# SCUT-CCNL/3DSIFT

Measured on AMD Instinct MI355X. Metric: Mvoxels/s end-to-end KpSiftAlgorithm on 512^3 fp32, higher is better.
Workload: dtype f32

## Files before the change

3dsift_amd/csrc/context.hip:

```cpp
#include <float.h>
#include <math.h>
#include <stdlib.h>
#include <string.h>

#include <algorithm>
#include <atomic>
#include <mutex>
#include <thread>

#include "ctx_internal.h"

#pragma clang fp contract(off)

namespace s3d {

static thread_local std::string g_last_error;
void set_last_error(const std::string &s) { g_last_error = s; }

int set_device(int device) {
	int n = 0;
	if (hipGetDeviceCount(&n) != hipSuccess || n <= 0) {
		set_last_error("no HIP device visible: this library has no CPU fallback");
		return SIFT3D_ERR_NO_DEVICE;
	}
// ... 31 lines not shown
		int *base = nullptr;
		S3D_HIP(hipMalloc(&base, sizeof(int) * words));
		hipError_t me = hipMemsetAsync(base, 0, sizeof(int) * words, c->stream);
		if (me == hipSuccess) me = hipStreamSynchronize(c->stream);
		if (me != hipSuccess) {
			hipFree(base);
			set_last_error(std::string("HIP error: ") + hipGetErrorString(me) + " (clearing the split-window scratch)");
			return SIFT3D_ERR_HIP;
		}
		c->dsplit.gacc = base;
		c->dsplit.gmass = reinterpret_cast<float *>(base + (size_t)scap * kDesc);
		c->dsplit.gdone = reinterpret_cast<unsigned *>(base + (size_t)scap * (kDesc + 8));
		c->dsplit.cap = scap;
	}
	S3D_HIP(hipMalloc(&c->d_prov, sizeof(unsigned) * ((size_t)c->ext_cap + 1)));
	c->det.prov = c->d_prov; c->det.prov_count = c->d_prov + c->ext_cap; c->det.prov_cap = c->ext_cap;
	if (c->det_o.size() > 1) {
		const size_t n2 = c->det_o.size() - 1;
		const unsigned slice = std::max(64u, (unsigned)(c->ext_cap / n2));
		S3D_HIP(hipMalloc(&c->d_prov2, sizeof(unsigned) * ((size_t)slice + 1) * n2));
		for (size_t o = 1; o < c->det_o.size(); o++) {
			c->det_o[o].prov = c->d_prov2 + (o - 1) * ((size_t)slice + 1);
			c->det_o[o].prov_count = c->det_o[o].prov + slice;
			c->det_o[o].prov_cap = slice;
		}
	}
	return SIFT3D_OK;
}

extern "C" void sift3d_default_params(sift3d_params *p) {
	if (!p) return;
	p->num_kp_levels = 3;
	p->sigma_default = 1.6f;
	p->sigma_n_default = 1.15f;
	p->peak_thresh = 0.1f;
	p->max_eig_thres = 0.9f;
	p->corner_thresh = 0.4f;
}
// ... 215 lines not shown
		CHECKED(hipMalloc(&c->arena, sizeof(float) * total));
	}
	float *p = c->arena;
	if (c->in_own) c->in.d = c->in_own;
	else { c->in.d = p; p += al64(c->in.n()); }
	c->tmpA.assign((size_t)std::max(1, c->noct), nullptr);
	c->tmpB.assign((size_t)std::max(1, c->noct), nullptr);
	for (int o = 0; o < c->noct && !c->slab; o++) {
		const size_t vo = al64(c->gss[(size_t)o * c->ng].n());
		c->tmpA[o] = p; p += vo;
		c->tmpB[o] = p; p += vo;
	}
	for (auto &L : c->gss) { L.d = p; p += al64(L.n()); }
	for (auto &L : c->dog) { L.d = p; p += al64(L.n()); }

	const size_t nwords = 1 + (size_t)std::max(1, c->noct * c->nd) + 8 + 1;
	CHECKED(hipMalloc(&c->d_words, sizeof(unsigned) * nwords));
	CHECKED(hipMemset(c->d_words, 0, sizeof(unsigned) * nwords));
	CHECKED(hipHostMalloc(&c->h_words, sizeof(unsigned) * 8, hipHostMallocDefault));
	CHECKED(hipMalloc(&c->d_slots_part, sizeof(unsigned) * slots_scratch_words()));
	c->d_inmax = c->d_words;
	c->d_dogmax = c->d_words + 1;
	c->d_total = c->d_words + 1 + std::max(1, c->noct * c->nd);
	c->d_nkp = c->d_total + 2;

	const int scan_planes = c->slab ? (c->own1 - c->own0) : cfg.nz;
	{
		const size_t kl = (size_t)c->p.num_kp_levels;
		const size_t words = kl * (size_t)scan_planes * cfg.ny * ((cfg.nx + 63) / 64);
		c->det_blocks = kl * (size_t)scan_planes * ((cfg.ny + 15) / 16);
		CHECKED(hipMalloc(&c->det.masks, sizeof(unsigned long long) * std::max<size_t>(words, 1)));
		CHECKED(hipMalloc(&c->det.block_counts, sizeof(unsigned) * std::max<size_t>(c->det_blocks, 1)));
		CHECKED(hipMalloc(&c->det.block_offsets, sizeof(unsigned) * std::max<size_t>(c->det_blocks, 1)));
	}
	c->det.total = c->d_total;
	{
		const bool det_serial = hook(SIFT3D_HOOK_DET_SERIAL) != 0;
		if (!c->slab && c->noct > 1 && !det_serial && c->ostream.size() > 1 && c->ostream[1] != c->stream) {
// ... 63 lines not shown
extern "C" int sift3d_create(sift3d_handle *out, const float *volume, int nx, int ny, int nz, const sift3d_params *params,
                             int device, int volume_on_device) {
	if (!out || !volume || nx <= 0 || ny <= 0 || nz <= 0) { set_last_error("sift3d_create: bad argument"); return SIFT3D_ERR_ARG; }
	if ((size_t)nx * ny * nz >= ((size_t)1 << 31)) { set_last_error("volume too large for int32 voxel indices"); return SIFT3D_ERR_ARG; }
	CreateCfg cfg;
	cfg.nx = nx; cfg.ny = ny; cfg.nz = nz;
	if (!volume_on_device) cfg.host_volume = volume;
	int rc = create_common(out, cfg, params, device);
	if (rc) return rc;
	sift3d_ctx *c = *out;
	const size_t V0 = (size_t)nx * ny * nz;
	hipError_t e = hipSuccess;
	if (volume_on_device) e = hipMemcpyAsync(c->in.d, volume, sizeof(float) * V0, hipMemcpyDeviceToDevice, c->stream);
	else if ((rc = join_upload(c)) != SIFT3D_OK) { sift3d_destroy(c); *out = nullptr; return rc; }
	if (e == hipSuccess) {
		unsigned *d_nonfinite = c->d_words + 1 + (size_t)std::max(1, c->noct * c->nd) + 8;
		launch_absmax(c->in.d, V0, c->d_inmax, c->stream, d_nonfinite);
		launch_scale_by_max(c->in.d, V0, c->d_inmax, c->stream);
		e = hipMemcpyAsync(&c->h_words[7], d_nonfinite, sizeof(unsigned), hipMemcpyDeviceToHost, c->stream);
		if (e == hipSuccess) e = hipStreamSynchronize(c->stream);
		if (e == hipSuccess && c->h_words[7] != 0) { c->nonfinite = true; c->use_fused = false; }
	}
	if (e == hipSuccess) e = hipGetLastError();
	if (e != hipSuccess) { set_last_error(hipGetErrorString(e)); sift3d_destroy(c); *out = nullptr; return SIFT3D_ERR_HIP; }
	return SIFT3D_OK;
}

#ifndef S3D_FUSED_MIN_DEFAULT
#define S3D_FUSED_MIN_DEFAULT 33
#endif
#ifndef S3D_O0_TAIL_SLOTS_DEFAULT
// ... 209 lines not shown

static int enqueue_detect(sift3d_ctx *c, const RunPlan &plan, int upto) {
	hipStream_t st = c->stream, sb = plan_stream(c, plan.det_two ? 1 : 0), sc = plan_stream(c, plan.det_rest_stream);
	std::vector<DetectLevels> DLs((size_t)c->noct);
	const int nl = c->nd - 2;
	const Taps *lt = c->g_last_elide ? &c->taps[c->ng - 1] : nullptr;
	DetectOpts dopt;
	dopt.neighbours = c->dopt.neighbours; dopt.refine = c->dopt.refine;
	dopt.max_offset = c->dopt.max_offset; dopt.contrast_thresh = c->dopt.contrast_thresh; dopt.edge_ratio = c->dopt.edge_ratio;
	const DetectOpts *dop = c->run_full ? &dopt : nullptr;
	if (upto >= 3)
		for (int o = 0; o < c->noct; o++) fill_detect_levels(c, o, DLs[(size_t)o]);
	auto bufs = [&](int o) -> const DetectBufs & { return plan.det_two && o > 0 ? c->det_o[(size_t)o] : c->det; };
	auto mark = [&](int o, hipStream_t s) {
		const Level &C = c->dog[(size_t)o * c->nd + 1];
		launch_detect_mark(DLs[(size_t)o], nl, C.nx, C.ny, C.zr_all(), c->p.peak_thresh, o + c->octave_base, bufs(o), s, lt, dop);
	};
	hipStream_t join = plan.det_early ? sb : st;
	if (plan.det_early) {
		S3D_HIP(hipEventRecord(c->ev_det_fork, st));
		mark(0, st);
		S3D_HIP(hipStreamWaitEvent(sb, c->ev_det_fork, 0));
	}
	for (int o = 1; o < c->noct; o++) S3D_HIP(hipStreamWaitEvent(join, c->ev_done[(size_t)o], 0));
	S3D_HIP(hipEventRecord(c->ev[1], join));
	S3D_HIP(hipEventRecord(c->ev[2], join));
	if (upto < 3) return SIFT3D_OK;
	if (plan.det_two) {
		for (int o = 1; o < c->noct; o++) {
			if (plan.det_rest_own && o >= 2) S3D_HIP(hipStreamWaitEvent(sc, c->ev_done[(size_t)o], 0));
			mark(o, o == 1 ? sb : sc);
// ... 7 lines not shown
		if (!plan.det_two) mark(o, st);
		if (plan.det_two && o == 1) {
			S3D_HIP(hipStreamWaitEvent(st, c->ev_det_join, 0));
			if (sc != sb) S3D_HIP(hipStreamWaitEvent(st, c->ev_det_join2, 0));
		}
		if (plan.emit == kEmitMultiAll || (plan.emit == kEmitMultiRest && o > 0)) multi.push_back(DetectEmitItem{&DLs[(size_t)o], nl, C.nx, C.ny, C.zr_all(), o + c->octave_base, &bufs(o)});
		else launch_detect_emit(DLs[(size_t)o], nl, C.nx, C.ny, C.zr_all(), o + c->octave_base, bufs(o), c->d_ext, c->ext_cap, st);
	}
	if (!multi.empty()) launch_detect_emit_multi(multi.data(), (int)multi.size(), c->d_ext, c->ext_cap, c->d_total, st);
	return SIFT3D_OK;
}

void enqueue_slots(sift3d_ctx *c) {
	launch_slots(c->d_ext, c->d_codes, c->d_total, c->ext_cap, c->d_nkp, c->d_order, c->kp_cap, c->d_slots_part, c->stream);
}
void enqueue_orient(sift3d_ctx *c, int rank, int world) {
	launch_orient(c->d_ext, c->d_codes, c->d_total, c->ext_cap, c->d_levels, c->d_luts, c->d_lutpool, c->p.max_eig_thres, c->p.corner_thresh,
	              rank, world, c->d_order, c->d_nkp + 3, c->stream);
	enqueue_slots(c);
}
void enqueue_describe(sift3d_ctx *c, int rank, int world, bool with_desc) {
	if (with_desc)
		launch_describe(c->d_ext, c->d_total, c->ext_cap, c->d_levels, c->d_luts, c->d_lutpool, c->d_desc, c->kp_cap, rank, world, c->d_order,
		                c->d_nkp, c->d_nkp + 1, c->stream, c->desc_lut_lds, &c->dsplit);
	launch_finalize(c->d_ext, c->d_total, c->ext_cap, with_desc, c->d_kpout, c->d_xyz, c->kp_cap, c->stream);
}

static int run_scratch(sift3d_ctx *c, int upto) {
	if (c->run_refine && upto >= 4 && c->refined_cap < c->kp_cap) {
		hipFree(c->d_refined); c->d_refined = nullptr; c->refined_cap = 0;
		S3D_HIP(hipMalloc(&c->d_refined, sizeof(sift3d_refined) * (size_t)c->kp_cap));
		c->refined_cap = c->kp_cap;
	}
	if (c->dsplit_dirty && c->dsplit.gacc) {
		S3D_HIP(hipMemsetAsync(c->dsplit.gacc, 0, sizeof(int) * (size_t)c->dsplit.cap * (kDesc + 8 + 1), c->stream));
		c->dsplit_dirty = false;
	}
	return SIFT3D_OK;
}

static int run_enqueue(sift3d_ctx *c, int upto, bool part_orient) {
	int rc = set_device(c->device);
	if (rc) return rc;
	if ((rc = run_scratch(c, upto)) != SIFT3D_OK) return rc;
	hipStream_t st = c->stream;
	const RunPlan &plan = c->plan;
	if (c->gate) { S3D_HIP(hipStreamWaitEvent(st, c->gate, 0)); c->gate = nullptr; }
	S3D_HIP(hipMemsetAsync(c->d_dogmax, 0, sizeof(unsigned) * (size_t)(std::max(1, c->noct * c->nd) + 6), st));
	S3D_HIP(hipEventRecord(c->ev[0], st));
	if ((rc = enqueue_pyramid(c, plan)) != SIFT3D_OK) return rc;
	if ((rc = enqueue_detect(c, plan, upto)) != SIFT3D_OK) return rc;
	S3D_HIP(hipEventRecord(c->ev[3], st));
	if (upto >= 4) enqueue_orient(c, part_orient ? c->part_rank : 0, part_orient ? c->part_world : 1);
	S3D_HIP(hipEventRecord(c->ev[4], st));
	if (upto >= 4) enqueue_describe(c, c->part_rank, c->part_world, upto >= 5);
	if (upto >= 4 && c->run_refine) {
		DogTable T;
		fill_dog_table(c, T);
		launch_refine(c->d_ext, c->d_total, c->ext_cap, c->kp_cap, T, c->p.num_kp_levels, c->d_refined, st);
	}
	S3D_HIP(hipEventRecord(c->ev[5], st));
	S3D_HIP(hipMemcpyAsync(c->h_words, c->d_total, sizeof(unsigned) * 5, hipMemcpyDeviceToHost, st));
	return SIFT3D_OK;
}


static int run_finish(sift3d_ctx *c, int upto, bool &again) {
	again = false;
	int rc = set_device(c->device);
	if (rc) return rc;
// ... 295 lines not shown
```

3dsift_amd/csrc/ctx_internal.h:

```cpp
#pragma once

#include <string>
#include <thread>
#include <vector>

#include "sift3d_internal.h"

using s3d::DescSplit; using s3d::DetectBufs; using s3d::DevKp; using s3d::Level; using s3d::LevelRef; using s3d::Taps; using s3d::WinLut;


constexpr int kChainStream = -1;
enum { kEmitPerOctave = 0, kEmitMultiRest = 1, kEmitMultiAll = 2 };
struct RunPlan {
	struct Oct {
		int head = 0, tail = 0;
		bool tail_moved = false;
		int prio = 0;
		int head_slots = 0, tail_slots = 0;
	};
	std::vector<Oct> oct;
	bool chain = false;
	int small_first = -1;
	s3d::SmallArgs small{};
	bool det_two = false;
// ... 26 lines not shown
	float *in_own = nullptr;
	void *in_raw = nullptr;
	hipStream_t up_stream = nullptr;
	std::thread uploader;
	int upload_rc = SIFT3D_OK;
	std::string upload_err;
	size_t arena_floats = 0;
	Level in;
	std::vector<Level> gss, dog;
	std::vector<float *> tmpA, tmpB;
	std::vector<hipStream_t> ostream;
	hipStream_t cstream = nullptr;
	std::vector<hipEvent_t> ev_seed, ev_done;
	hipEvent_t ev_fork = nullptr;
	unsigned *d_words = nullptr;
	unsigned *d_slots_part = nullptr;
	unsigned *h_words = nullptr;
	unsigned *d_inmax = nullptr, *d_dogmax = nullptr, *d_total = nullptr, *d_nkp = nullptr;
	DetectBufs det{};
	size_t det_blocks = 0;
	std::vector<DetectBufs> det_o;
	unsigned long long *d_masks2 = nullptr;
	unsigned *d_counts2 = nullptr, *d_offsets2 = nullptr, *d_prov2 = nullptr;
	hipEvent_t ev_det_fork = nullptr, ev_det_join = nullptr, ev_det_join2 = nullptr;
	DevKp *d_ext = nullptr;
	int *d_codes = nullptr, *d_order = nullptr;
	unsigned ext_cap = 0, kp_cap = 0;
	LevelRef *d_levels = nullptr;
	WinLut *d_luts = nullptr;
	float *d_lutpool = nullptr;
// ... 40 lines not shown
	size_t ext_arena_floats = 0;
};

namespace s3d {
bool build_taps(float sigma, Taps &t);
void level_sigmas(const sift3d_params &p, std::vector<float> &sig, float &base_sigma);
void build_faces(FaceConst *F);
bool build_facesym(const FaceConst *F, FaceSym *S);
bool append_lut(std::vector<float> &pool, WinLut &L, int which, float sigma, float radius, float u, float scale);
int set_device(int device);
int alloc_lists(sift3d_ctx *c, unsigned ext_cap);
float level_scale(const sift3d_params &p, int octave, int s);
void plan_pyramid(sift3d_ctx *c, int noct_total);
void fill_detect_levels(const sift3d_ctx *c, int o, DetectLevels &DL);
void enqueue_slots(sift3d_ctx *c);
void enqueue_orient(sift3d_ctx *c, int rank, int world);
void enqueue_describe(sift3d_ctx *c, int rank, int world, bool with_desc);
int upload_luts(sift3d_ctx *c, const std::vector<WinLut> &luts, std::vector<float> &pool);
std::vector<WinLut> blank_luts(const sift3d_ctx *c);
size_t arena_floats_of(const sift3d_ctx *c);
int create_common(sift3d_handle *out, const CreateCfg &cfg, const sift3d_params *params, int device);
int join_upload(sift3d_ctx *c);
int run_impl(sift3d_ctx *c, int upto, bool part_orient = false);
}
```

3dsift_amd/csrc/kernels_desc.hip:

```cpp
#include <float.h>

#include <stdio.h>

#include <algorithm>

#include "sift3d_internal.h"

namespace s3d {

__constant__ FaceConst c_faces[kFaces];
__constant__ FaceSym c_sym;

hipError_t upload_faces(const FaceConst *faces, const FaceSym *sym) {
	hipError_t e = hipMemcpyToSymbol(HIP_SYMBOL(c_faces), faces, sizeof(FaceConst) * kFaces);
	if (e == hipSuccess) e = hipMemcpyToSymbol(HIP_SYMBOL(c_sym), sym, sizeof(FaceSym));
	return e;
}

__device__ __forceinline__ void win_bounds_d(float c, float rad, float u, int n, int &lo, int &hi) {
	int s = (int)floorf(c - __fdiv_rn(rad, u));
	lo = s > 1 ? s : 1;
	int e = (int)ceilf(c + __fdiv_rn(rad, u));
	hi = e < (n - 2) ? e : n - 2;
}
// ... 822 lines not shown
	int total = 0;
	for (int i = 0; i < kDesc; i++) total += marks[i] != 0u;
	float n2 = 0.0f;
	for (int i = 0; i < total; i++) n2 = n2 + trunc_thresh * trunc_thresh;
	const float cn = (float)((double)sqrtf(n2) + DBL_EPSILON);
	const float cv = trunc_thresh * (float)(1.0 / (double)cn);
	for (int i = tid; i < kDesc; i += 256) row[i] = marks[i] != 0u ? cv : 0.0f;
}
void launch_describe_overflow(const DevKp *kps, unsigned k, const LevelRef *d_levels, const WinLut *d_luts, const float *d_lutpool, float *d_desc,
                              hipStream_t st) {
	hipLaunchKernelGGL(k_describe_overflow, dim3(1), dim3(256), 0, st, kps, k, d_levels, d_luts, d_lutpool, d_desc);
}

void launch_describe(const DevKp *kps, const unsigned *d_count, unsigned cap, const LevelRef *d_levels, const WinLut *d_luts,
                     const float *d_lutpool, float *d_desc, unsigned kp_cap, int part_rank, int part_world, const int *order,
                     const unsigned *d_nkp, unsigned *d_work, hipStream_t st, bool lut_in_lds, const DescSplit *split) {
	(void)hipMemsetAsync(d_work, 0, 2 * sizeof(unsigned), st);
	DescSplit sp{};
	if (split && split->gacc && lut_in_lds && !hook(SIFT3D_HOOK_DESC_NOSPLIT)) sp = *split;
	static const int desc_grid = dev_tune_i("S3D_DESC_GRID", 256 * 8);
	const int dev_flags = (hook(SIFT3D_HOOK_DESC_NOCACHE) ? 1 : 0) | (hook(SIFT3D_HOOK_DESC_EXACT_CELLS) ? 2 : 0) | (hook(SIFT3D_HOOK_DESC_MASS_SHIFT) & 63) << 8;
	const unsigned wide_hi = kWideBelow, wide_lo = sp.gacc ? std::min(kSplit4Below, wide_hi) : 0u;
	if (lut_in_lds) {
		hipLaunchKernelGGL((k_describe<true, 256>), dim3(desc_grid), dim3(256), 0, st, kps, d_count, cap, d_levels, d_luts, d_lutpool, d_desc, kp_cap,
		                   part_rank, part_world, order, d_nkp, d_work, dev_flags, wide_lo, wide_hi, sp, DescPartial{});
		if (wide_hi > wide_lo)
			hipLaunchKernelGGL((k_describe<true, 512>), dim3(256 * 2), dim3(512), 0, st, kps, d_count, cap, d_levels, d_luts, d_lutpool, d_desc, kp_cap,
			                   part_rank, part_world, order, d_nkp, d_work, dev_flags, wide_lo, wide_hi, DescSplit{}, DescPartial{});
	} else {
		hipLaunchKernelGGL((k_describe<false, 256>), dim3(256 * 8), dim3(256), 0, st, kps, d_count, cap, d_levels, d_luts, d_lutpool, d_desc, kp_cap,
		                   part_rank, part_world, order, d_nkp, d_work, dev_flags, 0u, 0u, DescSplit{}, DescPartial{});
	}
// ... 124 lines not shown
```

3dsift_amd/csrc/kernels_detect.hip:

```cpp
#include <stdio.h>
#include <string.h>
#include <stdlib.h>

#include <algorithm>

#include "sift3d_internal.h"

namespace s3d {

#ifndef S3D_DETDIAG
#define S3D_DETDIAG 0
#endif
constexpr int kRows = 32;
constexpr int kThreads = 256;

constexpr int kQueue = 640;
__global__ void __launch_bounds__(kThreads) k_mark(DetectLevels L, int nx, int ny, ZRange zr, int nyb, float peak_thresh,
                                                   unsigned long long *__restrict__ masks, unsigned *__restrict__ block_counts,
                                                   unsigned *__restrict__ prov, unsigned *__restrict__ prov_count, unsigned prov_cap,
                                                   unsigned *__restrict__ total) {
	__shared__ unsigned s_cnt[kThreads / 64];
	__shared__ uint2 s_q[kThreads / 64][kQueue];
	extern __shared__ unsigned long long s_mask_dyn[];
	const int segw = min((nx + 63) >> 6, 64);
	const int b = blockIdx.x;
	const int nz = zr.zo1 - zr.zo0;
	const int yb = b % nyb, zi = (b / nyb) % nz, lvl = b / (nyb * nz);
	const int z = zr.zo0 + zi;
	const int zg = z + zr.zoff;
	const float *__restrict__ cur = L.cur[lvl];
	const float *__restrict__ prev = L.prev[lvl];
	const float *__restrict__ next = L.next[lvl];
	const bool lazy_prev = lvl == 0 && L.prev0_hi != nullptr, lazy_next = lvl == L.nextl_slot && L.nextl_hi != nullptr;
	const bool lazy_g = lvl == L.nextl_slot && L.lazy_src != nullptr;
	const float thr = peak_thresh * __uint_as_float(*L.absmax_bits[lvl]);
	const int wpr = (nx + 63) >> 6;
	const int lane = threadIdx.x & 63, wid = threadIdx.x >> 6;
	const size_t sy = (size_t)nx, sz = (size_t)nx * ny;
	const bool z_in = (zg >= 1 && zg <= zr.nzg - 2);
	const int y0 = yb * kRows;
	constexpr int kBatch = 8;
	const int nrows = min(kRows, ny - y0);
	const int swid = __builtin_amdgcn_readfirstlane(wid);
	const int r_lo = swid * (kRows / 4), r_hi = min(nrows, (swid + 1) * (kRows / 4));
	uint2 *q = s_q[swid];
	unsigned long long *mloc = s_mask_dyn + (size_t)swid * (kRows / 4) * segw;
	for (int i = lane; i < (kRows / 4) * segw; i += 64) mloc[i] = 0ull;
	const unsigned long long lt = (1ull << lane) - 1ull;
	const size_t plane0 = sz * (size_t)z + sy * (size_t)y0;
	int qn = 0;
	auto evaluate = [&](int first, int n, int seg0) {
		if (S3D_DETDIAG & 1) {
			const uint2 qd = q[first + min(lane, n - 1)];
			if (lane < n && __uint_as_float(qd.x) == 12345.678f) atomicOr(&mloc[0], 1ull);
			return;
		}
// ... 26 lines not shown
					else total[1] = 1u;
				}
			}
			return;
		}
		const float n7 = lazy_next ? (L.nextl_hi[ic] - L.nextl_lo[ic]) * (-1.0f) : next[ic];
		const bool mn = !dmax && v < n0 && v < n5 && v < n6 && v < n7;
		const bool mx = dmax && v > n0 && v > n5 && v > n6 && v > n7;
		if (act && (mn || mx)) atomicOr(&mloc[rr * segw + xw], 1ull << bit);
	};
	unsigned cnt = 0;
	for (int seg0 = 0; seg0 < wpr; seg0 += 64) {
		const int seg1 = min(wpr, seg0 + 64);
		if (z_in) {
			const int ry_a = max(r_lo, 1 - y0), ry_b = min(r_hi, ny - 1 - y0);
			const int nws = seg1 - seg0;
			const float *__restrict__ pl = cur + sz * (size_t)z + (size_t)seg0 * 64;
			auto word = [&](float v, float u, float d, float xl, float xr, int wseg, unsigned idrow) {
				const float hi = fmaxf(fmaxf(u, d), fmaxf(xl, xr)), lo = fminf(fminf(u, d), fminf(xl, xr));
				const bool gmax = v > hi;
				const bool c = fabsf(v) > thr && (gmax || v < lo) && !((S3D_DETDIAG & 2) && v != 12345.678f);
				const unsigned long long m = __ballot(c);
				if (c) {
					const unsigned pos = __builtin_amdgcn_mbcnt_hi((unsigned)(m >> 32), __builtin_amdgcn_mbcnt_lo((unsigned)m, (unsigned)qn));
					q[pos] = make_uint2(__float_as_uint(v), idrow | (gmax ? 0x10000u : 0u) | (unsigned)(wseg << 6) | (unsigned)lane);
				}
				qn += (int)__popcll(m);
			};
			const unsigned omax = (unsigned)(nx - 1 - seg0 * 64);
			for (int w0 = 0; w0 < nws && ry_a < ry_b; w0 += kBatch) {
				unsigned off[kBatch];
#pragma unroll
				for (int bb = 0; bb < kBatch; bb++) off[bb] = min((unsigned)(min(w0 + bb, nws - 1) * 64 + lane), omax);
				const int eoff = (lane & 1) ? (int)min((unsigned)((w0 + kBatch) * 64), omax) : w0 * 64 - 1;
				float up[kBatch], mid[kBatch], emid;
				{
					const float *ra = pl + sy * (size_t)(y0 + ry_a - 1), *rb = ra + sy;
#pragma unroll
					for (int bb = 0; bb < kBatch; bb++) { up[bb] = ra[off[bb]]; mid[bb] = rb[off[bb]]; }
					emid = rb[eoff];
				}
				for (int ry = ry_a; ry < ry_b; ry++) {
					const float *rd = pl + sy * (size_t)(y0 + ry + 1);
					float dn[kBatch], xl[kBatch], xr[kBatch];
#pragma unroll
					for (int bb = 0; bb < kBatch; bb++) dn[bb] = rd[off[bb]];
					const float edn = rd[eoff];
#pragma unroll
					for (int bb = 0; bb < kBatch; bb++) {
						const int le = __builtin_amdgcn_readlane(__float_as_int(bb == 0 ? emid : mid[bb > 0 ? bb - 1 : 0]), bb == 0 ? 0 : 63);
						const int re = __builtin_amdgcn_readlane(__float_as_int(bb == kBatch - 1 ? emid : mid[bb < kBatch - 1 ? bb + 1 : 0]), bb == kBatch - 1 ? 1 : 0);
						xl[bb] = __int_as_float(__builtin_amdgcn_update_dpp(le, __float_as_int(mid[bb]), 0x138 , 0xf, 0xf, false));
						xr[bb] = __int_as_float(__builtin_amdgcn_update_dpp(re, __float_as_int(mid[bb]), 0x130 , 0xf, 0xf, false));
					}
					const unsigned idrow = (unsigned)((ry - r_lo) << 12);
#pragma unroll
					for (int bb = 0; bb < kBatch; bb++)
						if (w0 + bb < nws) word(mid[bb], up[bb], dn[bb], xl[bb], xr[bb], w0 + bb, idrow);
					while (qn >= 64) {
						qn -= 64;
						evaluate(qn, 64, seg0);
					}
#pragma unroll
					for (int bb = 0; bb < kBatch; bb++) { up[bb] = mid[bb]; mid[bb] = dn[bb]; }
					emid = edn;
				}
			}
		}
		if (qn > 0) evaluate(0, qn, seg0);
		qn = 0;
		for (int ry = r_lo; ry < r_hi; ry++) {
			unsigned long long *mrow = masks + ((size_t)(lvl * nz + zi) * ny + (y0 + ry)) * wpr;
			for (int xw = seg0 + lane; xw < seg1; xw += 64) {
				const unsigned long long m = mloc[(ry - r_lo) * segw + xw - seg0];
				mrow[xw] = m;
				cnt += (unsigned)__popcll(m);
				mloc[(ry - r_lo) * segw + xw - seg0] = 0ull;
			}
		}
	}
#pragma unroll
// ... 371 lines not shown
                                                   int octave, DetectLevels L, DevKp *__restrict__ out, unsigned cap,
                                                   unsigned *__restrict__ total) {
	__shared__ unsigned s_wave[kThreads / 64];
	emit_block((int)blockIdx.x, masks, block_offsets, nx, ny, zr, nyb, octave, L.level_id, L.scale, out, cap, total, s_wave);
}

__global__ void __launch_bounds__(kThreads) k_emit_multi(EmitMulti M, DevKp *__restrict__ out, unsigned cap, unsigned *__restrict__ total) {
	__shared__ unsigned s_wave[kThreads / 64];
	int k = 0;
	while (k + 1 < M.n && blockIdx.x >= M.o[k + 1].block0) k++;
	const EmitOct &E = M.o[k];
	emit_block((int)(blockIdx.x - E.block0), E.masks, E.offsets, E.nx, E.ny, E.zr, E.nyb, E.octave, E.level_id, E.scale, out, cap, total, s_wave);
}

void launch_detect_mark(const DetectLevels &L, int nlevels, int nx, int ny, const ZRange &zr, float peak_thresh, int octave,
                        const DetectBufs &b, hipStream_t st, const Taps *lazy_taps, const DetectOpts *opt) {
	if (opt) { launch_mark_full(L, nlevels, nx, ny, zr, kRows, peak_thresh, *opt, b, st); return; }
	const int nyb = (ny + kRows - 1) / kRows;
	const int nzl = zr.zo1 - zr.zo0;
	if (nzl <= 0) return;
	const unsigned nblocks = (unsigned)(nlevels * nzl * nyb);
	if (nblocks == 0) return;
	const bool lazy = L.lazy_src != nullptr && lazy_taps != nullptr && b.prov != nullptr;
	if (lazy) (void)hipMemsetAsync(b.prov_count, 0, sizeof(unsigned), st);
	const size_t mask_lds = sizeof(unsigned long long) * (kThreads / 64) * (kRows / 4) * (size_t)std::min((nx + 63) >> 6, 64);
	hipLaunchKernelGGL(k_mark, dim3(nblocks), dim3(kThreads), mask_lds, st, L, nx, ny, zr, nyb, peak_thresh, b.masks, b.block_counts, b.prov,
	                   b.prov_count, b.prov_cap, b.total);
	if (lazy) {
		const bool wave_form = lazy_taps->hw == 8 && !hook(SIFT3D_HOOK_LAZY_GENERIC) && (size_t)nx * (size_t)ny * 17u * sizeof(float) < ((size_t)1 << 32);
		auto grid = [&](unsigned full, unsigned per_wg) { return dim3(std::max(1u, std::min(full, (nblocks + per_wg - 1) / per_wg))); };
		if (wave_form)
			hipLaunchKernelGGL(k_lazy_wave, grid(256 * 3, kLwWaves), dim3(64 * kLwWaves), 0, st, L, *lazy_taps, nx, ny, zr, nyb, b.prov, b.prov_count, b.prov_cap,
			                   b.masks, b.block_counts);
		if (2 * lazy_taps->hw + 1 <= 17)
			hipLaunchKernelGGL(k_lazy_next<17>, grid(wave_form ? 1536 : 1024, 1), dim3(256), 0, st, L, *lazy_taps, nx, ny, zr, nyb, b.prov, b.prov_count, b.prov_cap,
			                   b.masks, b.block_counts, wave_form ? 1 : 0);
		else
			hipLaunchKernelGGL(k_lazy_next<25>, grid(512, 1), dim3(256), 0, st, L, *lazy_taps, nx, ny, zr, nyb, b.prov, b.prov_count, b.prov_cap,
			                   b.masks, b.block_counts, 0);
// ... 46 lines not shown
```

3dsift_amd/csrc/kernels_orient.hip:

```cpp
#include <float.h>

#include "sift3d_internal.h"

namespace s3d {

__device__ __forceinline__ float wave_sum(float v) {
#pragma unroll
	for (int o = 32; o > 0; o >>= 1) v = v + __shfl_xor(v, o, 64);
	return v;
}

__device__ __forceinline__ void win_bounds(float c, float rad, float u, int n, int &lo, int &hi) {
	int s = (int)floorf(c - __fdiv_rn(rad, u));
	lo = s > 1 ? s : 1;
	int e = (int)ceilf(c + __fdiv_rn(rad, u));
	hi = e < (n - 2) ? e : n - 2;
}

__device__ void eig_sym3(const double A[9], double w[3], double V[9]) {
	double a[9];
#pragma unroll
	for (int i = 0; i < 9; i++) { a[i] = A[i]; V[i] = (i % 4 == 0) ? 1.0 : 0.0; }
	for (int sweep = 0; sweep < 64; sweep++) {
		const double off = fabs(a[1]) + fabs(a[2]) + fabs(a[5]);
// ... 379 lines not shown
		const float T6[6] = {kp.st[0], kp.st[1], kp.st[2], kp.st[4], kp.st[5], kp.st[8]};
		const float w3[3] = {kp.win[0], kp.win[1], kp.win[2]};
		bool near = false;
		kp.code = finish_orientation(kp, T6, w3, max_eig, corner, &near);
		kps[k] = kp;
		codes[k] = kp.code == 1 ? ((kp.level << 4) | 1) : kp.code;
		if (!pass && near) {
			const unsigned pos = atomicAdd(redo_count, 1u);
			if (pos < cap) redo_list[pos] = (int)k;
		}
	}
}

void launch_orient(DevKp *kps, int *codes, const unsigned *d_count, unsigned cap, const LevelRef *d_levels, const WinLut *d_luts,
                   const float *d_lutpool, float max_eig, float corner, int part_rank, int part_world, int *redo_list, unsigned *redo_count,
                   hipStream_t st) {
	static const int dflt_grid = dev_tune_i("S3D_ORI_GRID", 256 * 32);
	const int ori_grid = hook(SIFT3D_HOOK_ORI_GRID) > 0 ? hook(SIFT3D_HOOK_ORI_GRID) : dflt_grid;
	(void)hipMemsetAsync(redo_count, 0, sizeof(unsigned), st);
	hipLaunchKernelGGL(k_orient<false>, dim3(ori_grid), dim3(256), 0, st, kps, codes, d_count, cap, d_levels, d_luts, d_lutpool, max_eig, corner,
	                   part_rank, part_world, (const int *)redo_list, (const unsigned *)redo_count);
	hipLaunchKernelGGL(k_orient_finish, dim3(256 * 8), dim3(64), 0, st, kps, codes, d_count, cap, max_eig, corner, part_rank, part_world, 0,
	                   redo_list, redo_count);
	hipLaunchKernelGGL(k_orient<true>, dim3(ori_grid), dim3(256), 0, st, kps, codes, d_count, cap, d_levels, d_luts, d_lutpool, max_eig, corner,
	                   part_rank, part_world, (const int *)redo_list, (const unsigned *)redo_count);
	hipLaunchKernelGGL(k_orient_finish, dim3(256 * 2), dim3(64), 0, st, kps, codes, d_count, cap, max_eig, corner, part_rank, part_world, 1,
	                   redo_list, redo_count);
}

static_assert(offsetof(DevKp, st) + sizeof(float) * 9 - offsetof(DevKp, win) == sizeof(float) * (kOrientWords - 1), "DevKp layout");

__global__ void __launch_bounds__(256) k_orient_pack(const DevKp *__restrict__ kps, const unsigned *__restrict__ d_count, unsigned cap,
                                                     int *__restrict__ dst, int part_rank, int part_world) {
	const unsigned count = min(d_count[0], cap);
// ... 133 lines not shown
```

3dsift_amd/csrc/sift3d_internal.h:

```cpp
#pragma once

#include <hip/hip_runtime.h>
#include <stdint.h>

#include <string>
#include <vector>

#include "../../include/sift3d_hip.h"
#include "../../include/sift3d_hip_test.h"

#pragma clang fp contract(off)

namespace s3d {

#ifndef S3D_MAX_HW
#define S3D_MAX_HW 64
#endif
constexpr int kMaxHW = S3D_MAX_HW;
constexpr int kMaxTaps = 2 * kMaxHW + 1;
constexpr int kDesc = SIFT3D_DESC_NUMEL;
constexpr int kFaces = 20;

struct Taps {
	int hw;
// ... 110 lines not shown
	const float *cur[kMaxKpLevels], *prev[kMaxKpLevels], *next[kMaxKpLevels];
	const float *prev0_hi, *prev0_lo;
	const float *nextl_hi, *nextl_lo;
	int nextl_slot;
	const float *lazy_src;
	const unsigned *absmax_bits[kMaxKpLevels];
	int level_id[kMaxKpLevels];
	float scale[kMaxKpLevels];
};
constexpr int kLazySlots = 52;
struct DetectOpts {
	int neighbours = 8, refine = 0;
	float max_offset = 0.5f, contrast_thresh = 0.0f, edge_ratio = 0.0f;
};
void launch_detect_mark(const DetectLevels &L, int nlevels, int nx, int ny, const ZRange &zr, float peak_thresh, int octave,
                        const DetectBufs &b, hipStream_t st, const Taps *lazy_taps, const DetectOpts *opt = nullptr);
void launch_mark_full(const DetectLevels &L, int nlevels, int nx, int ny, const ZRange &zr, int rows, float peak_thresh, const DetectOpts &opt,
                      const DetectBufs &b, hipStream_t st);
constexpr int kDogTabOct = 12, kDogTabLv = 8;
struct DogTable {
	const float *d[kDogTabOct][kDogTabLv];
	int nx[kDogTabOct], ny[kDogTabOct];
	int octave_base;
};
void launch_detect_emit(const DetectLevels &L, int nlevels, int nx, int ny, const ZRange &zr, int octave, const DetectBufs &b, DevKp *out,
                        unsigned cap, hipStream_t st);
struct DetectEmitItem { const DetectLevels *L; int nlevels, nx, ny; ZRange zr; int octave; const DetectBufs *b; };
void launch_detect_emit_multi(const DetectEmitItem *items, int n, DevKp *out, unsigned cap, unsigned *total, hipStream_t st);
void launch_detect_octave(const DetectLevels &L, int nlevels, int nx, int ny, const ZRange &zr, float peak_thresh, int octave,
                          const DetectBufs &b, DevKp *out, unsigned cap, hipStream_t st, const Taps *lazy_taps = nullptr);

#ifdef __HIPCC__
typedef const float __attribute__((address_space(1))) *gfloat_p;
__device__ __forceinline__ gfloat_p as_global(const float *p) { return (gfloat_p)p; }
#endif

struct LevelRef {
	const float *d;
	int nx, ny, nz;
	float unit;
	int zoff;
};
void launch_orient(DevKp *kps, int *codes, const unsigned *d_count, unsigned cap, const LevelRef *d_levels ,
                   const WinLut *d_luts, const float *d_lutpool, float max_eig, float corner, int part_rank, int part_world,
                   int *redo_list , unsigned *redo_count,
                   hipStream_t st);
constexpr int kOrientWords = 34;
void launch_orient_pack(const DevKp *kps, const unsigned *d_count, unsigned cap, int *dst, int part_rank, int part_world, hipStream_t st);
void launch_orient_unpack(DevKp *kps, int *codes, const unsigned *d_count, unsigned cap, const int *src, hipStream_t st);
size_t slots_scratch_words();
void launch_slots(DevKp *kps, const int *codes, const unsigned *d_count, unsigned cap, unsigned *d_nkp, int *order, unsigned kp_cap,
                  unsigned *scratch, hipStream_t st);

hipError_t upload_faces(const FaceConst *faces, const FaceSym *sym);
struct DescSplit {
	int *gacc = nullptr;
	float *gmass = nullptr;
	unsigned *gdone = nullptr;
	unsigned cap = 0;
};
constexpr int kDescSegs = 6;
// ... 7 lines not shown
};
struct DescPartial {
	int zc0 = 0, zc1 = 0, nseg = 0;
	int H[8] = {0, 0, 0, 0, 0, 0, 0, 0};
	DescSeg seg[kDescSegs];
};
void launch_export_records(const DevKp *ext, const int *order, unsigned n, DevKp *dst, hipStream_t st);
void launch_describe_partial(const LevelRef *d_levels, const WinLut *d_luts, const float *d_lutpool, const DescPartial &pp,
                             unsigned *d_work , hipStream_t st, bool lut_in_lds = true);
void launch_describe_finish(const DevKp *recs, unsigned n, const LevelRef *d_levels, const WinLut *d_luts, int nparts, const int *const *d_hist, const float *const *d_mass,
                            const float *d_units, bool final_round, float *d_desc, int *d_redo, float *d_units_next, unsigned *d_counters,
                            hipStream_t st);
void launch_describe(const DevKp *kps, const unsigned *d_count, unsigned cap, const LevelRef *d_levels,
                     const WinLut *d_luts, const float *d_lutpool, float *d_desc, unsigned kp_cap, int part_rank, int part_world,
                     const int *order, const unsigned *d_nkp, unsigned *d_work ,
                     hipStream_t st, bool lut_in_lds = true, const DescSplit *split = nullptr);
void launch_face_lookup(const float *d_g3, int n, int route, int *d_face, float *d_bary3, hipStream_t st);
void launch_refine(const DevKp *kps, const unsigned *d_count, unsigned cap, unsigned kp_cap, const DogTable &T, int num_kp_levels,
                   sift3d_refined *out, hipStream_t st);
void launch_finalize(const DevKp *kps, const unsigned *d_count, unsigned cap, int transposed,
                     sift3d_keypoint *d_out, float *d_xyz, unsigned kp_cap, hipStream_t st);

struct MatchGuard {
	float *s4; const float *a_n2; const unsigned *b_n2max; int *redo;
	bool small_offsets = false;
};
int match_rows_device(const float *d_a, const int *d_row_ids, int nrows, const float *d_b, int m, int *d_cand ,
                      void *d_part , float *d_gd, float *d_sd, int *d_gi, int *d_si, const MatchGuard &g, hipStream_t st);
size_t match_cand_bytes(size_t rows), match_part_bytes(size_t rows);
void launch_row_norm2(const float *d_a, int n, float *d_an2, const float *d_b, int m, float *d_bn2, unsigned *d_nmax, hipStream_t st);
int match_redo_rows();
// ... 146 lines not shown
```

Baseline: 19960.

## Fold per-stage counter memsets into one clear and vectorize detect-mark row scan

Gathers the provisional-keypoint counters into a parked block of the shared device word array. A single memset at the start of each run now clears that block, which lets the detect, orient and describe launches skip their own small hipMemsetAsync calls. Separately, the k_mark extremum scan is rewritten to use buffer-resource 128-bit loads over 256-wide spans with a three-row rotating register window. It adds v_max3/v_min3 inline asm and an early skip for wavefronts where no value passes the threshold. This trades per-launch memset overhead and scalar loads for more complex code and register pressure.

New measurement: 20360, median of 6. +2.0%, better.

```diff
diff --git a/3dsift_amd/csrc/context.hip b/3dsift_amd/csrc/context.hip
--- a/3dsift_amd/csrc/context.hip
+++ b/3dsift_amd/csrc/context.hip
@@ -69,14 +69,14 @@
 		c->dsplit.cap = scap;
 	}
 	S3D_HIP(hipMalloc(&c->d_prov, sizeof(unsigned) * ((size_t)c->ext_cap + 1)));
-	c->det.prov = c->d_prov; c->det.prov_count = c->d_prov + c->ext_cap; c->det.prov_cap = c->ext_cap;
+	c->det.prov = c->d_prov; c->det.prov_count = c->d_parked; c->det.prov_cap = c->ext_cap;
 	if (c->det_o.size() > 1) {
 		const size_t n2 = c->det_o.size() - 1;
 		const unsigned slice = std::max(64u, (unsigned)(c->ext_cap / n2));
 		S3D_HIP(hipMalloc(&c->d_prov2, sizeof(unsigned) * ((size_t)slice + 1) * n2));
 		for (size_t o = 1; o < c->det_o.size(); o++) {
 			c->det_o[o].prov = c->d_prov2 + (o - 1) * ((size_t)slice + 1);
-			c->det_o[o].prov_count = c->det_o[o].prov + slice;
+			c->det_o[o].prov_count = c->d_parked + o;
 			c->det_o[o].prov_cap = slice;
 		}
 	}
@@ -322,14 +322,16 @@
 	for (auto &L : c->gss) { L.d = p; p += al64(L.n()); }
 	for (auto &L : c->dog) { L.d = p; p += al64(L.n()); }
 
-	const size_t nwords = 1 + (size_t)std::max(1, c->noct * c->nd) + 8 + 1;
+	const size_t nparked = (size_t)std::max(1, c->noct);
+	const size_t nwords = 1 + nparked + (size_t)std::max(1, c->noct * c->nd) + 8 + 1;
 	CHECKED(hipMalloc(&c->d_words, sizeof(unsigned) * nwords));
 	CHECKED(hipMemset(c->d_words, 0, sizeof(unsigned) * nwords));
 	CHECKED(hipHostMalloc(&c->h_words, sizeof(unsigned) * 8, hipHostMallocDefault));
 	CHECKED(hipMalloc(&c->d_slots_part, sizeof(unsigned) * slots_scratch_words()));
 	c->d_inmax = c->d_words;
-	c->d_dogmax = c->d_words + 1;
-	c->d_total = c->d_words + 1 + std::max(1, c->noct * c->nd);
+	c->d_parked = c->d_words + 1;
+	c->d_dogmax = c->d_parked + nparked;
+	c->d_total = c->d_dogmax + std::max(1, c->noct * c->nd);
 	c->d_nkp = c->d_total + 2;
 
 	const int scan_planes = c->slab ? (c->own1 - c->own0) : cfg.nz;
@@ -423,7 +425,7 @@
 	if (volume_on_device) e = hipMemcpyAsync(c->in.d, volume, sizeof(float) * V0, hipMemcpyDeviceToDevice, c->stream);
 	else if ((rc = join_upload(c)) != SIFT3D_OK) { sift3d_destroy(c); *out = nullptr; return rc; }
 	if (e == hipSuccess) {
-		unsigned *d_nonfinite = c->d_words + 1 + (size_t)std::max(1, c->noct * c->nd) + 8;
+		unsigned *d_nonfinite = c->d_total + 8;
 		launch_absmax(c->in.d, V0, c->d_inmax, c->stream, d_nonfinite);
 		launch_scale_by_max(c->in.d, V0, c->d_inmax, c->stream);
 		e = hipMemcpyAsync(&c->h_words[7], d_nonfinite, sizeof(unsigned), hipMemcpyDeviceToHost, c->stream);
@@ -663,7 +665,7 @@
 	auto bufs = [&](int o) -> const DetectBufs & { return plan.det_two && o > 0 ? c->det_o[(size_t)o] : c->det; };
 	auto mark = [&](int o, hipStream_t s) {
 		const Level &C = c->dog[(size_t)o * c->nd + 1];
-		launch_detect_mark(DLs[(size_t)o], nl, C.nx, C.ny, C.zr_all(), c->p.peak_thresh, o + c->octave_base, bufs(o), s, lt, dop);
+		launch_detect_mark(DLs[(size_t)o], nl, C.nx, C.ny, C.zr_all(), c->p.peak_thresh, o + c->octave_base, bufs(o), s, lt, dop, plan.det_two || o == 0);
 	};
 	hipStream_t join = plan.det_early ? sb : st;
 	if (plan.det_early) {
@@ -701,15 +703,15 @@
 void enqueue_slots(sift3d_ctx *c) {
 	launch_slots(c->d_ext, c->d_codes, c->d_total, c->ext_cap, c->d_nkp, c->d_order, c->kp_cap, c->d_slots_part, c->stream);
 }
-void enqueue_orient(sift3d_ctx *c, int rank, int world) {
+void enqueue_orient(sift3d_ctx *c, int rank, int world, bool counters_clear) {
 	launch_orient(c->d_ext, c->d_codes, c->d_total, c->ext_cap, c->d_levels, c->d_luts, c->d_lutpool, c->p.max_eig_thres, c->p.corner_thresh,
-	              rank, world, c->d_order, c->d_nkp + 3, c->stream);
+	              rank, world, c->d_order, c->d_nkp + 3, c->stream, counters_clear);
 	enqueue_slots(c);
 }
-void enqueue_describe(sift3d_ctx *c, int rank, int world, bool with_desc) {
+void enqueue_describe(sift3d_ctx *c, int rank, int world, bool with_desc, bool counters_clear) {
 	if (with_desc)
 		launch_describe(c->d_ext, c->d_total, c->ext_cap, c->d_levels, c->d_luts, c->d_lutpool, c->d_desc, c->kp_cap, rank, world, c->d_order,
-		                c->d_nkp, c->d_nkp + 1, c->stream, c->desc_lut_lds, &c->dsplit);
+		                c->d_nkp, c->d_nkp + 1, c->stream, c->desc_lut_lds, &c->dsplit, counters_clear);
 	launch_finalize(c->d_ext, c->d_total, c->ext_cap, with_desc, c->d_kpout, c->d_xyz, c->kp_cap, c->stream);
 }
 
@@ -733,14 +735,14 @@
 	hipStream_t st = c->stream;
 	const RunPlan &plan = c->plan;
 	if (c->gate) { S3D_HIP(hipStreamWaitEvent(st, c->gate, 0)); c->gate = nullptr; }
-	S3D_HIP(hipMemsetAsync(c->d_dogmax, 0, sizeof(unsigned) * (size_t)(std::max(1, c->noct * c->nd) + 6), st));
+	S3D_HIP(hipMemsetAsync(c->d_parked, 0, sizeof(unsigned) * (size_t)(c->d_total + 6 - c->d_parked), st));
 	S3D_HIP(hipEventRecord(c->ev[0], st));
 	if ((rc = enqueue_pyramid(c, plan)) != SIFT3D_OK) return rc;
 	if ((rc = enqueue_detect(c, plan, upto)) != SIFT3D_OK) return rc;
 	S3D_HIP(hipEventRecord(c->ev[3], st));
-	if (upto >= 4) enqueue_orient(c, part_orient ? c->part_rank : 0, part_orient ? c->part_world : 1);
+	if (upto >= 4) enqueue_orient(c, part_orient ? c->part_rank : 0, part_orient ? c->part_world : 1, true);
 	S3D_HIP(hipEventRecord(c->ev[4], st));
-	if (upto >= 4) enqueue_describe(c, c->part_rank, c->part_world, upto >= 5);
+	if (upto >= 4) enqueue_describe(c, c->part_rank, c->part_world, upto >= 5, true);
 	if (upto >= 4 && c->run_refine) {
 		DogTable T;
 		fill_dog_table(c, T);
diff --git a/3dsift_amd/csrc/ctx_internal.h b/3dsift_amd/csrc/ctx_internal.h
--- a/3dsift_amd/csrc/ctx_internal.h
+++ b/3dsift_amd/csrc/ctx_internal.h
@@ -64,6 +64,7 @@
 	std::vector<hipEvent_t> ev_seed, ev_done;
 	hipEvent_t ev_fork = nullptr;
 	unsigned *d_words = nullptr;
+	unsigned *d_parked = nullptr;
 	unsigned *d_slots_part = nullptr;
 	unsigned *h_words = nullptr;
 	unsigned *d_inmax = nullptr, *d_dogmax = nullptr, *d_total = nullptr, *d_nkp = nullptr;
@@ -134,8 +135,8 @@
 void plan_pyramid(sift3d_ctx *c, int noct_total);
 void fill_detect_levels(const sift3d_ctx *c, int o, DetectLevels &DL);
 void enqueue_slots(sift3d_ctx *c);
-void enqueue_orient(sift3d_ctx *c, int rank, int world);
-void enqueue_describe(sift3d_ctx *c, int rank, int world, bool with_desc);
+void enqueue_orient(sift3d_ctx *c, int rank, int world, bool counters_clear = false);
+void enqueue_describe(sift3d_ctx *c, int rank, int world, bool with_desc, bool counters_clear = false);
 int upload_luts(sift3d_ctx *c, const std::vector<WinLut> &luts, std::vector<float> &pool);
 std::vector<WinLut> blank_luts(const sift3d_ctx *c);
 size_t arena_floats_of(const sift3d_ctx *c);
diff --git a/3dsift_amd/csrc/kernels_desc.hip b/3dsift_amd/csrc/kernels_desc.hip
--- a/3dsift_amd/csrc/kernels_desc.hip
+++ b/3dsift_amd/csrc/kernels_desc.hip
@@ -860,8 +860,8 @@
 
 void launch_describe(const DevKp *kps, const unsigned *d_count, unsigned cap, const LevelRef *d_levels, const WinLut *d_luts,
                      const float *d_lutpool, float *d_desc, unsigned kp_cap, int part_rank, int part_world, const int *order,
-                     const unsigned *d_nkp, unsigned *d_work, hipStream_t st, bool lut_in_lds, const DescSplit *split) {
-	(void)hipMemsetAsync(d_work, 0, 2 * sizeof(unsigned), st);
+                     const unsigned *d_nkp, unsigned *d_work, hipStream_t st, bool lut_in_lds, const DescSplit *split, bool work_is_clear) {
+	if (!work_is_clear) (void)hipMemsetAsync(d_work, 0, 2 * sizeof(unsigned), st);
 	DescSplit sp{};
 	if (split && split->gacc && lut_in_lds && !hook(SIFT3D_HOOK_DESC_NOSPLIT)) sp = *split;
 	static const int desc_grid = dev_tune_i("S3D_DESC_GRID", 256 * 8);
diff --git a/3dsift_amd/csrc/kernels_detect.hip b/3dsift_amd/csrc/kernels_detect.hip
--- a/3dsift_amd/csrc/kernels_detect.hip
+++ b/3dsift_amd/csrc/kernels_detect.hip
@@ -3,6 +3,7 @@
 #include <stdlib.h>
 
 #include <algorithm>
+#include <type_traits>
 
 #include "sift3d_internal.h"
 
@@ -15,6 +16,9 @@
 constexpr int kThreads = 256;
 
 constexpr int kQueue = 640;
+constexpr int kSpans = 2;
+typedef float f4m __attribute__((ext_vector_type(4)));
+typedef unsigned u4m __attribute__((ext_vector_type(4)));
 __global__ void __launch_bounds__(kThreads) k_mark(DetectLevels L, int nx, int ny, ZRange zr, int nyb, float peak_thresh,
                                                    unsigned long long *__restrict__ masks, unsigned *__restrict__ block_counts,
                                                    unsigned *__restrict__ prov, unsigned *__restrict__ prov_count, unsigned prov_cap,
@@ -39,7 +43,6 @@
 	const size_t sy = (size_t)nx, sz = (size_t)nx * ny;
 	const bool z_in = (zg >= 1 && zg <= zr.nzg - 2);
 	const int y0 = yb * kRows;
-	constexpr int kBatch = 8;
 	const int nrows = min(kRows, ny - y0);
 	const int swid = __builtin_amdgcn_readfirstlane(wid);
 	const int r_lo = swid * (kRows / 4), r_hi = min(nrows, (swid + 1) * (kRows / 4));
@@ -96,57 +99,91 @@
 		const int seg1 = min(wpr, seg0 + 64);
 		if (z_in) {
 			const int ry_a = max(r_lo, 1 - y0), ry_b = min(r_hi, ny - 1 - y0);
-			const int nws = seg1 - seg0;
-			const float *__restrict__ pl = cur + sz * (size_t)z + (size_t)seg0 * 64;
-			auto word = [&](float v, float u, float d, float xl, float xr, int wseg, unsigned idrow) {
-				const float hi = fmaxf(fmaxf(u, d), fmaxf(xl, xr)), lo = fminf(fminf(u, d), fminf(xl, xr));
-				const bool gmax = v > hi;
-				const bool c = fabsf(v) > thr && (gmax || v < lo) && !((S3D_DETDIAG & 2) && v != 12345.678f);
-				const unsigned long long m = __ballot(c);
-				if (c) {
-					const unsigned pos = __builtin_amdgcn_mbcnt_hi((unsigned)(m >> 32), __builtin_amdgcn_mbcnt_lo((unsigned)m, (unsigned)qn));
-					q[pos] = make_uint2(__float_as_uint(v), idrow | (gmax ? 0x10000u : 0u) | (unsigned)(wseg << 6) | (unsigned)lane);
+			const int nsp = (seg1 - seg0 + 3) >> 2, X0 = seg0 * 64;
+			const unsigned row_bytes = (unsigned)sizeof(float) * (unsigned)nx;
+			const __amdgpu_buffer_rsrc_t rows = __builtin_amdgcn_make_buffer_rsrc(
+				const_cast<float *>(cur + sz * (size_t)z + sy * (size_t)(y0 + ry_a - 1) - 1), 0,
+				(int)std::min<size_t>(0xFFFFFFFFull, sizeof(float) * (sy * (size_t)max(ry_b - ry_a + 2, 0) + 4)), 0x00020000);
+			const unsigned lpc = (unsigned)min(4 * lane, ((min(nx, 256) - 1) >> 2) << 2);
+			auto pass = [&](auto ns, int s0) {
+				constexpr int NS = decltype(ns)::value;
+				unsigned voff[NS], eoff[NS], xid[NS];
+				unsigned long long vm[NS][4];
+#pragma unroll
+				for (int sb = 0; sb < NS; sb++) {
+					const int A = X0 + 256 * (s0 + sb), S = nx >= 256 ? min(A, nx - 256) : 0;
+					voff[sb] = 4u * (1u + (unsigned)S + lpc);
+					eoff[sb] = 4u * (unsigned)(lane == 63 ? min(S + 256, nx - 1) + 1 : S);
+					xid[sb] = (unsigned)(S - X0 + 4 * lane);
+#pragma unroll
+					for (int c = 0; c < 4; c++) {
+						const int x = S + 4 * lane + c;
+						vm[sb][c] = __ballot(x >= max(A, 1) && x <= nx - 2);
+					}
 				}
-				qn += (int)__popcll(m);
-			};
-			const unsigned omax = (unsigned)(nx - 1 - seg0 * 64);
-			for (int w0 = 0; w0 < nws && ry_a < ry_b; w0 += kBatch) {
-				unsigned off[kBatch];
-#pragma unroll
-				for (int bb = 0; bb < kBatch; bb++) off[bb] = min((unsigned)(min(w0 + bb, nws - 1) * 64 + lane), omax);
-				const int eoff = (lane & 1) ? (int)min((unsigned)((w0 + kBatch) * 64), omax) : w0 * 64 - 1;
-				float up[kBatch], mid[kBatch], emid;
-				{
-					const float *ra = pl + sy * (size_t)(y0 + ry_a - 1), *rb = ra + sy;
-#pragma unroll
-					for (int bb = 0; bb < kBatch; bb++) { up[bb] = ra[off[bb]]; mid[bb] = rb[off[bb]]; }
-					emid = rb[eoff];
-				}
-				for (int ry = ry_a; ry < ry_b; ry++) {
-					const float *rd = pl + sy * (size_t)(y0 + ry + 1);
-					float dn[kBatch], xl[kBatch], xr[kBatch];
-#pragma unroll
-					for (int bb = 0; bb < kBatch; bb++) dn[bb] = rd[off[bb]];
-					const float edn = rd[eoff];
-#pragma unroll
-					for (int bb = 0; bb < kBatch; bb++) {
-						const int le = __builtin_amdgcn_readlane(__float_as_int(bb == 0 ? emid : mid[bb > 0 ? bb - 1 : 0]), bb == 0 ? 0 : 63);
-						const int re = __builtin_amdgcn_readlane(__float_as_int(bb == kBatch - 1 ? emid : mid[bb < kBatch - 1 ? bb + 1 : 0]), bb == kBatch - 1 ? 1 : 0);
-						xl[bb] = __int_as_float(__builtin_amdgcn_update_dpp(le, __float_as_int(mid[bb]), 0x138 , 0xf, 0xf, false));
-						xr[bb] = __int_as_float(__builtin_amdgcn_update_dpp(re, __float_as_int(mid[bb]), 0x130 , 0xf, 0xf, false));
+				auto load_row = [&](int ry, f4m (&v)[NS], float (&e)[NS], bool edges) {
+					const int roff = (int)((unsigned)(ry - (ry_a - 1)) * row_bytes);
+#pragma unroll
+					for (int sb = 0; sb < NS; sb++) {
+							const u4m p = __builtin_amdgcn_raw_buffer_load_b128(rows, (int)voff[sb], roff, 0);
+							v[sb] = f4m{__uint_as_float(p.x), __uint_as_float(p.y), __uint_as_float(p.z), __uint_as_float(p.w)};
+							if (edges) e[sb] = __uint_as_float(__builtin_amdgcn_raw_buffer_load_b32(rows, (int)eoff[sb], roff, 0));
+						}
+				};
+				auto comp = [&](float v, float u, float d, float xl, float xr, unsigned long long m, unsigned id) {
+					float hi, lo;
+					asm("v_max3_f32 %0, %1, %2, %3\n\tv_max_f32 %0, %0, %4" : "=&v"(hi) : "v"(u), "v"(d), "v"(xl), "v"(xr));
+					asm("v_min3_f32 %0, %1, %2, %3\n\tv_min_f32 %0, %0, %4" : "=&v"(lo) : "v"(u), "v"(d), "v"(xl), "v"(xr));
+					const bool gmax = v > hi;
+					m &= __ballot(fabsf(v) > thr) & (__ballot(gmax) | __ballot(v < lo));
+					if (S3D_DETDIAG & 2) m &= __ballot(v == 12345.678f);
+					if (m) {
+						if (__builtin_amdgcn_inverse_ballot_w64(m)) {
+							const unsigned pos = __builtin_amdgcn_mbcnt_hi((unsigned)(m >> 32), __builtin_amdgcn_mbcnt_lo((unsigned)m, (unsigned)qn));
+							q[pos] = make_uint2(__float_as_uint(v), id | (gmax ? 0x10000u : 0u));
+						}
+						qn += (int)__popcll(m);
 					}
+				};
+				auto test_row = [&](const f4m (&up)[NS], const f4m (&mid)[NS], const float (&e)[NS], const f4m (&dn)[NS], int ry) {
 					const unsigned idrow = (unsigned)((ry - r_lo) << 12);
 #pragma unroll
-					for (int bb = 0; bb < kBatch; bb++)
-						if (w0 + bb < nws) word(mid[bb], up[bb], dn[bb], xl[bb], xr[bb], w0 + bb, idrow);
+					for (int sb = 0; sb < NS; sb++) {
+							const f4m v = mid[sb], u = up[sb], d = dn[sb];
+							float t;
+							asm("v_max3_f32 %0, |%1|, |%2|, |%3|\n\tv_max_f32 %0, %0, |%4|" : "=&v"(t) : "v"(v.x), "v"(v.y), "v"(v.z), "v"(v.w));
+							if (__ballot(t > thr) == 0ull) continue;
+							const float xl = __int_as_float(__builtin_amdgcn_update_dpp(__float_as_int(e[sb]), __float_as_int(v.w), 0x138 , 0xf, 0xf, false));
+							const float xr = __int_as_float(__builtin_amdgcn_update_dpp(__float_as_int(e[sb]), __float_as_int(v.x), 0x130 , 0xf, 0xf, false));
+							const unsigned id = idrow + xid[sb];
+							comp(v.x, u.x, d.x, xl, v.y, vm[sb][0], id);
+							comp(v.y, u.y, d.y, v.x, v.z, vm[sb][1], id + 1u);
+							comp(v.z, u.z, d.z, v.y, v.w, vm[sb][2], id + 2u);
+							comp(v.w, u.w, d.w, v.z, xr, vm[sb][3], id + 3u);
+						}
 					while (qn >= 64) {
 						qn -= 64;
 						evaluate(qn, 64, seg0);
 					}
-#pragma unroll
-					for (int bb = 0; bb < kBatch; bb++) { up[bb] = mid[bb]; mid[bb] = dn[bb]; }
-					emid = edn;
+				};
+				f4m ra[NS] = {}, rb[NS] = {}, rc[NS] = {};
+				float ea[NS] = {}, eb[NS] = {}, ec[NS] = {};
+				load_row(ry_a - 1, ra, ea, false);
+				load_row(ry_a, rb, eb, true);
+				for (int ry = ry_a; ry < ry_b; ry += 3) {
+					load_row(ry + 1, rc, ec, true);
+					test_row(ra, rb, eb, rc, ry);
+					if (ry + 1 >= ry_b) break;
+					load_row(ry + 2, ra, ea, true);
+					test_row(rb, rc, ec, ra, ry + 1);
+					if (ry + 2 >= ry_b) break;
+					load_row(ry + 3, rb, eb, true);
+					test_row(rc, ra, ea, rb, ry + 2);
 				}
+			};
+			for (int s0 = 0; s0 < nsp && ry_a < ry_b; s0 += kSpans) {
+				if (s0 + 1 < nsp) pass(std::integral_constant<int, kSpans>{}, s0);
+				else pass(std::integral_constant<int, 1>{}, s0);
 			}
 		}
 		if (qn > 0) evaluate(0, qn, seg0);
@@ -548,7 +585,7 @@
 }
 
 void launch_detect_mark(const DetectLevels &L, int nlevels, int nx, int ny, const ZRange &zr, float peak_thresh, int octave,
-                        const DetectBufs &b, hipStream_t st, const Taps *lazy_taps, const DetectOpts *opt) {
+                        const DetectBufs &b, hipStream_t st, const Taps *lazy_taps, const DetectOpts *opt, bool parked_is_clear) {
 	if (opt) { launch_mark_full(L, nlevels, nx, ny, zr, kRows, peak_thresh, *opt, b, st); return; }
 	const int nyb = (ny + kRows - 1) / kRows;
 	const int nzl = zr.zo1 - zr.zo0;
@@ -556,7 +593,7 @@
 	const unsigned nblocks = (unsigned)(nlevels * nzl * nyb);
 	if (nblocks == 0) return;
 	const bool lazy = L.lazy_src != nullptr && lazy_taps != nullptr && b.prov != nullptr;
-	if (lazy) (void)hipMemsetAsync(b.prov_count, 0, sizeof(unsigned), st);
+	if (lazy && !parked_is_clear) (void)hipMemsetAsync(b.prov_count, 0, sizeof(unsigned), st);
 	const size_t mask_lds = sizeof(unsigned long long) * (kThreads / 64) * (kRows / 4) * (size_t)std::min((nx + 63) >> 6, 64);
 	hipLaunchKernelGGL(k_mark, dim3(nblocks), dim3(kThreads), mask_lds, st, L, nx, ny, zr, nyb, peak_thresh, b.masks, b.block_counts, b.prov,
 	                   b.prov_count, b.prov_cap, b.total);
diff --git a/3dsift_amd/csrc/kernels_orient.hip b/3dsift_amd/csrc/kernels_orient.hip
--- a/3dsift_amd/csrc/kernels_orient.hip
+++ b/3dsift_amd/csrc/kernels_orient.hip
@@ -417,10 +417,10 @@
 
 void launch_orient(DevKp *kps, int *codes, const unsigned *d_count, unsigned cap, const LevelRef *d_levels, const WinLut *d_luts,
                    const float *d_lutpool, float max_eig, float corner, int part_rank, int part_world, int *redo_list, unsigned *redo_count,
-                   hipStream_t st) {
+                   hipStream_t st, bool count_is_clear) {
 	static const int dflt_grid = dev_tune_i("S3D_ORI_GRID", 256 * 32);
 	const int ori_grid = hook(SIFT3D_HOOK_ORI_GRID) > 0 ? hook(SIFT3D_HOOK_ORI_GRID) : dflt_grid;
-	(void)hipMemsetAsync(redo_count, 0, sizeof(unsigned), st);
+	if (!count_is_clear) (void)hipMemsetAsync(redo_count, 0, sizeof(unsigned), st);
 	hipLaunchKernelGGL(k_orient<false>, dim3(ori_grid), dim3(256), 0, st, kps, codes, d_count, cap, d_levels, d_luts, d_lutpool, max_eig, corner,
 	                   part_rank, part_world, (const int *)redo_list, (const unsigned *)redo_count);
 	hipLaunchKernelGGL(k_orient_finish, dim3(256 * 8), dim3(64), 0, st, kps, codes, d_count, cap, max_eig, corner, part_rank, part_world, 0,
diff --git a/3dsift_amd/csrc/sift3d_internal.h b/3dsift_amd/csrc/sift3d_internal.h
--- a/3dsift_amd/csrc/sift3d_internal.h
+++ b/3dsift_amd/csrc/sift3d_internal.h
@@ -148,7 +148,8 @@
 	float max_offset = 0.5f, contrast_thresh = 0.0f, edge_ratio = 0.0f;
 };
 void launch_detect_mark(const DetectLevels &L, int nlevels, int nx, int ny, const ZRange &zr, float peak_thresh, int octave,
-                        const DetectBufs &b, hipStream_t st, const Taps *lazy_taps, const DetectOpts *opt = nullptr);
+                        const DetectBufs &b, hipStream_t st, const Taps *lazy_taps, const DetectOpts *opt = nullptr,
+                        bool parked_is_clear = false );
 void launch_mark_full(const DetectLevels &L, int nlevels, int nx, int ny, const ZRange &zr, int rows, float peak_thresh, const DetectOpts &opt,
                       const DetectBufs &b, hipStream_t st);
 constexpr int kDogTabOct = 12, kDogTabLv = 8;
@@ -178,7 +179,7 @@
 void launch_orient(DevKp *kps, int *codes, const unsigned *d_count, unsigned cap, const LevelRef *d_levels ,
                    const WinLut *d_luts, const float *d_lutpool, float max_eig, float corner, int part_rank, int part_world,
                    int *redo_list , unsigned *redo_count,
-                   hipStream_t st);
+                   hipStream_t st, bool count_is_clear = false );
 constexpr int kOrientWords = 34;
 void launch_orient_pack(const DevKp *kps, const unsigned *d_count, unsigned cap, int *dst, int part_rank, int part_world, hipStream_t st);
 void launch_orient_unpack(DevKp *kps, int *codes, const unsigned *d_count, unsigned cap, const int *src, hipStream_t st);
@@ -216,7 +217,8 @@
 void launch_describe(const DevKp *kps, const unsigned *d_count, unsigned cap, const LevelRef *d_levels,
                      const WinLut *d_luts, const float *d_lutpool, float *d_desc, unsigned kp_cap, int part_rank, int part_world,
                      const int *order, const unsigned *d_nkp, unsigned *d_work ,
-                     hipStream_t st, bool lut_in_lds = true, const DescSplit *split = nullptr);
+                     hipStream_t st, bool lut_in_lds = true, const DescSplit *split = nullptr,
+                     bool work_is_clear = false );
 void launch_face_lookup(const float *d_g3, int n, int route, int *d_face, float *d_bary3, hipStream_t st);
 void launch_refine(const DevKp *kps, const unsigned *d_count, unsigned cap, unsigned kp_cap, const DogTable &T, int num_kp_levels,
                    sift3d_refined *out, hipStream_t st);
```
